# pcodec/pcodec

Measured on AMD Instinct MI355X. Metric: encode+decode GB/s (uncompressed) per chunk, u64/f64 2^18-elem, higher is better.
Workload: dtype u64

## Files before the change

### pcodec_amd/csrc/encode_fast.hip

```cpp
#pragma once

namespace pcogfx {

constexpr uint32_t kRunBatches = 64;

struct EncFast {
  uint8_t* sym;
  uint16_t* answ;
  uint32_t* bat;
  uint64_t* run_start;
  uint32_t* fstate;
  uint16_t* vlut;
  uint32_t bat_stride, run_stride;
  uint32_t runs_per_page, fused;
  uint64_t stride;
  uint64_t* body;
  uint32_t* wp_block;
};
__device__ __forceinline__ uint64_t fast_at(const EncPage PCO_GLOBAL* pg, uint32_t skip) { return uni((uint64_t)pg->start) + skip + 16ull * uni(pg->page_idx); }

__device__ __forceinline__ uint8_t PCO_GLOBAL* fsym_ptr(const EncWorkspace& ws, const EncFast& fx, uint32_t task, uint32_t var) {
  return (uint8_t PCO_GLOBAL*)fx.sym + ((uint64_t)task * ws.n_slots + ws.slot_of_var[var]) * fx.stride;
}
__device__ __forceinline__ uint16_t PCO_GLOBAL* fansw_ptr(const EncWorkspace& ws, const EncFast& fx, uint32_t task, uint32_t var) {
  return (uint16_t PCO_GLOBAL*)fx.answ + ((uint64_t)task * ws.n_slots + ws.slot_of_var[var]) * fx.stride;
}

struct PageVar { uint32_t present, n_bins, asl, max_ob, needs_ans, trivial, skip, n_lat, compact; uint64_t minv, rel, range; };
__device__ __forceinline__ PageVar page_var(const EncChunk PCO_GLOBAL* ch, uint32_t v, uint32_t page_n) {
  PageVar r;
  r.present = uni(ch->v[v].present); r.n_bins = uni(ch->v[v].n_bins); r.asl = uni(ch->v[v].ans_size_log); r.max_ob = uni(ch->v[v].max_ob);
  r.needs_ans = uni(ch->v[v].needs_ans); r.trivial = uni(ch->v[v].is_trivial);
// ... 628 lines not shown
  uint64_t bits = kBitsModeVariant;
  if (mode_kind == kIntMult || mode_kind == kFloatMult) bits += LB; else if (mode_kind == kFloatQuant) bits += kBitsQuantK;
  if (uni(ch->dict_dtype)) bits = 32 + 8ull * uni(ch->dict_k) * (uint32_t)(dtype_bits(uni(ch->dict_dtype)) / 8);
  bits += kBitsDeltaVariant;
  if (delta_kind == kDeltaConsecutive) bits += kBitsDeltaOrder + 1;
  else if (delta_kind == kDeltaLookback) bits += kBitsLookbackWindowLog + kBitsLookbackStateLog + 1;
  else if (delta_kind == kDeltaConv1) bits += 5 + 64 + 5 + 32ull * uni(ch->delta_order);
  for (int v = 0; v < 3; v++) {
    if (!uni(ch->v[v].present)) continue;
    const uint32_t lb = v == 0 ? 32u : LB;
    bits += kBitsAnsSizeLog + kBitsNBins + (uint64_t)uni(ch->v[v].n_bins) * (uni(ch->v[v].ans_size_log) + lb + offset_bits_bits(lb));
  }
  return (bits + 7) & ~(uint64_t)7;
}

__global__ __launch_bounds__(64) void enc_scan_kernel(EncWorkspace ws, EncFast fx, PcoGfxTaskResult* results, uint32_t n_pages) {
  const uint32_t p = blockIdx.x;
  if (p >= n_pages) return;
  const uint32_t lane = lane_id();
  EncPage PCO_GLOBAL* pg = (EncPage PCO_GLOBAL*)ws.pages + p;
  const uint32_t t = uni(pg->chunk);
  EncChunk PCO_GLOBAL* ch = (EncChunk PCO_GLOBAL*)ws.chunks + t;
  if (!page_is_fast(ch, pg)) return;
  const uint32_t LB = (uint32_t)dtype_bits(uni(ch->dtype));
  const uint32_t page_n = (uint32_t)uni((uint64_t)pg->n);
  const uint32_t pflags = uni(pg->flags);
  PageVar pv[3]; uint32_t ob0[3];
  uint64_t head = 0;
  if (pflags & kPageFlagPreamble) head += 8 + kBitsNEntries + chunk_meta_bits_of(ch, LB);
  uint64_t page_meta = 0;
  const uint32_t delta_kind = uni(ch->delta_kind);
#pragma unroll
  for (int v = 0; v < 3; v++) {
    pv[v] = page_var(ch, v, page_n);
    ob0[v] = 0;
    if (!pv[v].present) continue;
    if (pv[v].n_bins == 1) ob0[v] = uni((uint32_t)plan_ref(ws, t, v).bob()[0]);
    if (v == 1) page_meta += (uint64_t)LB * ((delta_kind == kDeltaConsecutive || delta_kind == kDeltaConv1) ? uni(ch->delta_order) : (delta_kind == kDeltaLookback ? (1u << uni(ch->state_n_log)) : 0u));
    page_meta += 4ull * pv[v].asl;
  }
  head += (page_meta + 7) & ~(uint64_t)7;
  uint32_t PCO_GLOBAL* dst32 = (uint32_t PCO_GLOBAL*)pg->dst;
  const uint64_t cap_bits = uni((uint64_t)pg->dst_cap) * 8;
  const uint32_t n_batches = (page_n + kBatchN - 1) / kBatchN;
  if (fx.body != nullptr) {
    const uint64_t rec = uni(fx.body[2ull * p]);
    if (rec >> 63) {
      const uint64_t end = head + (rec & ~(1ull << 63)), total = (end + 7) & ~(uint64_t)7;
      const bool overflow = total + 64 > cap_bits;
      if (lane == 0) {
        pg->pad = overflow ? 1u : (0x100u | (15u << 4));
        store_result((PcoGfxTaskResult PCO_GLOBAL*)results + p, overflow ? 0 : total >> 3, overflow ? PCO_GFX_INVALID_ARGUMENT : PCO_GFX_OK, 0);
        if (!overflow) { dst32[0] = 0; dst32[total >> 5] = 0; dst32[end >> 5] = 0; dst32[head >> 5] = 0; fx.run_start[(uint64_t)p * fx.run_stride] = head; }
      }
      return;
    }
  }
  uint64_t carry = head;
  for (int pass = 0; pass < 2; pass++) {
    carry = head;
    for (uint32_t c0 = 0; c0 < n_batches; c0 += 64) {
      const uint32_t b = c0 + lane;
      uint64_t bits = 0;
      if (b < n_batches) {
        const uint32_t base = b * kBatchN;
#pragma unroll
        for (int v = 0; v < 3; v++) {
          if (!pv[v].present || pv[v].trivial || base >= pv[v].n_lat) continue;
// ... 471 lines not shown
  if (kWide && (uint32_t)dtype_bits(uni(ch->dtype)) != LBits<L>::v) return;
  PageVar pv[3];
#pragma unroll
  for (int v = 0; v < 3; v++) pv[v] = page_var(ch, v, page_n);
  pack1_run<L, kMask, kWide>(ws, fx, p, run, pg, t, pv, page_n);
}

__global__ __launch_bounds__(64) void enc_pack_kernel(EncWorkspace ws, EncFast fx, uint32_t n_pages) {
  const uint32_t p = blockIdx.x / fx.runs_per_page, run = blockIdx.x % fx.runs_per_page;
  if (p >= n_pages) return;
  EncPage PCO_GLOBAL* pg = (EncPage PCO_GLOBAL*)ws.pages + p;
  EncChunk PCO_GLOBAL* ch = (EncChunk PCO_GLOBAL*)ws.chunks + uni(pg->chunk);
  const uint32_t pad = uni(pg->pad);
  if (!page_is_fast(ch, pg) || (pad & 1u) != 0) return;
  const bool lean = ((pad >> 4) & 0xfu) != 0;
  if (lean && run != 0) return;
  const int bits = dtype_bits(uni(ch->dtype));
  if (bits == 64) pack_run<uint64_t>(ws, fx, p, run, pg, ch, lean);
  else if (bits == 32) pack_run<uint32_t>(ws, fx, p, run, pg, ch, lean);
  else if (bits == 16) pack_run<uint16_t>(ws, fx, p, run, pg, ch, lean);
  else pack_run<uint8_t>(ws, fx, p, run, pg, ch, lean);
}

}
```

### pcodec_amd/csrc/encode_walkpack.hip

```cpp
#pragma once

namespace pcogfx {

constexpr uint32_t kWpWaves = 6;
constexpr uint32_t kWpQ = 16, kWpHelpers = 8, kWpH = kWpQ / kWpHelpers;
constexpr uint32_t kWpSlot = 5120;
constexpr uint32_t kWpStgDwords = 132;
constexpr uint32_t kWpSkew = 8, kWpSlotUse = kWpSlot - kWpSkew * (16 - 1);
__device__ __forceinline__ uint32_t wp_slot(uint32_t q) { return q * (kWpSlot + kWpSkew); }
constexpr uint32_t kWpStgOff = (kWpSlotUse - kWpStgDwords * 4) & ~15u;
constexpr uint32_t kWpAnsOff = kWpStgOff - 1024;
constexpr uint32_t kWpSymOff = kWpAnsOff - 512;
constexpr uint32_t kWpLdsBytes = kWpQ * kWpSlot;
static_assert(kWpStgOff % 16 == 0 && kWpAnsOff % 16 == 0 && kWpSymOff % 16 == 0 && kWpStgOff + kWpStgDwords * 4 <= kWpSlotUse, "aligned sections");
static_assert(2 * kWpLdsBytes <= 160 * 1024, "two blocks per CU");
constexpr uint64_t kWpBodyFlag = 1ull << 63;
__device__ __forceinline__ bool wp_fits(uint32_t asl, uint32_t n_bins) { return ew_info_off(asl) + 12u * n_bins <= kWpSymOff; }

__device__ __forceinline__ void wp_put(uint32_t stg_addr, uint32_t pos, uint64_t val) {
  const uint32_t dw = pos >> 5, sh = pos & 31;
  const uint64_t lo = val << sh;
  uint32_t PCO_LDS* s = (uint32_t PCO_LDS*)(uintptr_t)(stg_addr + 4u * dw);
  const uint32_t hi = (uint32_t)((val >> 1) >> (63 - sh));
  atomicOr((uint32_t*)&s[0], (uint32_t)lo);
// ... 5 lines not shown

__device__ __forceinline__ PageVar page_var_lane(const EncChunk PCO_GLOBAL* ch, uint32_t v, uint32_t page_n) {
  PageVar r;
  r.present = ch->v[v].present; r.n_bins = ch->v[v].n_bins; r.asl = ch->v[v].ans_size_log; r.max_ob = ch->v[v].max_ob;
  r.needs_ans = ch->v[v].needs_ans; r.trivial = ch->v[v].is_trivial;
  r.skip = v == 2 ? 0u : ch->v[v].lat_start;
  if (r.skip > page_n) r.skip = page_n;
  r.n_lat = page_n - r.skip;
  r.compact = ch->v[v].hist_path == 0 ? 1u : 0u;
  r.minv = (uint64_t)ch->v[v].minv;
  r.range = (uint64_t)ch->v[v].maxv - r.minv;
  r.rel = v != 0 && ch->c16_ok == 1 ? ch->c16_ref[v == 2 ? 1 : 0] : r.minv;
  return r;
}

__global__ __launch_bounds__(64 * (1 + kWpHelpers)) __attribute__((amdgpu_waves_per_eu(kWpWaves, kWpWaves))) void enc_walkp_kernel(EncWorkspace ws, EncFast fx, uint32_t n_pages) {
  const uint32_t lane = lane_id(), wave = threadIdx.x >> 6;
  uint8_t PCO_LDS* smem = enc_lds_base();
  const uint32_t lds0 = (uint32_t)(uintptr_t)smem;
  const uint32_t n_items = n_pages * ws.n_slots;
  typedef uint64_t __attribute__((aligned(2))) u64_align2;
  const uint32_t iq = lane & 15u, sub = lane >> 4;
  const uint32_t l_item = blockIdx.x * kWpQ + iq;
  const bool l_exists = l_item < n_items;
  const uint32_t l_p = l_exists ? l_item / ws.n_slots : 0u, l_sl = l_exists ? l_item % ws.n_slots : 0u;
  const uint32_t l_v = ws.slot_of_var[0] == l_sl ? 0u : (ws.slot_of_var[1] == l_sl ? 1u : 2u);
  const EncPage PCO_GLOBAL* l_pg = (const EncPage PCO_GLOBAL*)ws.pages + l_p;
  const uint32_t l_t = l_pg->chunk;
  const EncChunk PCO_GLOBAL* l_ch = (const EncChunk PCO_GLOBAL*)ws.chunks + l_t;
  const bool l_fast = l_exists && l_ch->status == PCO_GFX_OK && l_ch->fast_ok != 0 && !(l_pg->flags & kPageFlagMetaOnly);
  const uint32_t l_page_n = (uint32_t)l_pg->n;
  const PageVar l_pv = page_var_lane(l_ch, l_v, l_page_n);
  const bool l_writes = l_fast && l_pv.present && !l_pv.trivial;
  bool l_bad = false;
  if (l_writes) {
    if (l_v != 1 || !wd_walks(fx.fused, l_pv) || ws_walks(fx.fused, l_pv) || !wd_takes(fx.fused, l_pv) || !l_pv.needs_ans || l_pv.n_bins > 256 || !wp_fits(l_pv.asl, l_pv.n_bins)) l_bad = true;
    else if ((l_ch->v[0].present && !l_ch->v[0].is_trivial) || (l_ch->v[2].present && !l_ch->v[2].is_trivial)) l_bad = true;
  }
  {
    uint32_t worst = 0;
    if (l_writes && !l_bad) {
      const PlanRef plan = plan_ref(ws, l_t, l_v);
      for (uint32_t b = sub; b < l_pv.n_bins; b += 4) { const uint32_t w = ((plan.syminfo()[b] >> 14) & 15u) + 1u + plan.bob()[b]; worst = w > worst ? w : worst; }
    }
    { const uint32_t o = (uint32_t)__shfl_xor((int)worst, 16, 64); worst = worst > o ? worst : o; }
    { const uint32_t o = (uint32_t)__shfl_xor((int)worst, 32, 64); worst = worst > o ? worst : o; }
    if (worst > 16u) l_bad = true;
  }
  const bool ok = (fx.fused & kFusedLookups) != 0 && !__any(l_bad);
  if (threadIdx.x == 0) fx.wp_block[blockIdx.x] = ok ? 1u : 0u;
  if (!ok) {
    if (threadIdx.x < kWpQ) {
      const uint32_t item = blockIdx.x * kWpQ + threadIdx.x;
      if (item < n_items && ws.slot_of_var[1] == item % ws.n_slots) fx.body[2ull * (item / ws.n_slots)] = 0;
    }
    return;
  }
  const uint32_t l_nb = l_writes ? (l_pv.n_lat + kBatchN - 1) / kBatchN : 0u;
  const uint32_t max_nb = wave_max_u32(l_nb);
  if (l_fast && !l_writes && sub == 0 && wave == 0) {
    if (l_pv.present && (l_pv.n_bins <= 1 || l_pv.n_lat == 0)) for (uint32_t jj = 0; jj < 4; jj++) fx.fstate[((uint64_t)l_p * 3 + l_v) * 4 + jj] = 1u << l_pv.asl;
    if (l_v == 1) fx.body[2ull * l_p] = 0;
  }
  const uint32_t l_info_off = ew_info_off(l_pv.asl), l_cpk_off = l_info_off + 8u * l_pv.n_bins;
// ... 304 lines not shown
```

### pcodec_amd/csrc/pco_gfx.hip

```cpp
#include "pco_host.h"
#include "pco_half.h"

#include <algorithm>
#include <atomic>
#include <chrono>
#include <thread>
#include <mutex>
#include <condition_variable>
#include <functional>
#include <sched.h>
#include <pthread.h>
#include <sys/syscall.h>
#include <unistd.h>
#include <cstdlib>
#include <cstring>
#include <memory>
#include <unordered_map>

#include "pco_auto_host.inc"
#include "decode_kernel.hip"
#include "decode_trail.hip"
#include "encode_kernels.hip"
#include "encode_lookback.hip"
#include "encode_conv1.hip"
#include "encode_dict.hip"
#include "encode_hist_select.hip"
#include "encode_hist_literal.hip"
#include "auto_mode_kernels.hip"
#include "encode_fast.hip"
#include "encode_walkseg.hip"
#include "encode_walkpack.hip"
#include "stream_kernels.hip"
#include "stream_wrapped.hip"

namespace pcogfx {

static thread_local HostError g_err{PCO_GFX_OK, ""};
void set_error(int status, const std::string& msg) { g_err.status = status; g_err.msg = msg; }
void clear_error() { g_err.status = PCO_GFX_OK; g_err.msg.clear(); }

struct WorkspaceHolder {
  std::unordered_map<int, std::unique_ptr<Workspace>> by_device;
  ~WorkspaceHolder() {
    const bool worker = (long)syscall(SYS_gettid) != (long)getpid();
    for (auto& kv : by_device) {
      if (worker) { int cur = 0; const bool sw = hipGetDevice(&cur) == hipSuccess && cur != kv.first && hipSetDevice(kv.first) == hipSuccess; kv.second->release_all(); if (kv.second->last_event) (void)hipEventDestroy(kv.second->last_event); if (sw) (void)hipSetDevice(cur); }
// ... 521 lines not shown
```

### pcodec_amd/csrc/pco_gfx_encode_api.inc

```
namespace pcogfx {

struct ResolvedConfig {
  uint32_t level;
  uint32_t mode_kind; double mode_f64; uint64_t mode_u64;
  uint32_t delta_kind, delta_order;
  uint64_t max_page_n; bool enable_8_bit;
  bool strict_hist;
  bool conv1 = false;
  bool dict = false;
  DictTask* d_dict = nullptr;
  uint32_t unknown_flags = 0;
};

static bool g_strict_hist_env = env_is_one("PCO_GFX_STRICT_HISTOGRAM");
static ResolvedConfig resolve_config(const PcoChunkConfigEx* c) {
  ResolvedConfig r{8, PCO_MODE_AUTO, 0.0, 0, PCO_DELTA_AUTO, 0, 1u << 18, true, g_strict_hist_env};
  if (c) {
    r.level = c->compression_level; r.mode_kind = c->mode_kind; r.mode_f64 = c->mode_f64; r.mode_u64 = c->mode_u64;
    r.delta_kind = c->delta_kind; r.delta_order = c->delta_order; r.max_page_n = c->max_page_n ? c->max_page_n : (1u << 18);
    r.enable_8_bit = c->enable_8_bit != 0;
    r.strict_hist = g_strict_hist_env || (c->flags & PCO_GFX_CFG_STRICT_HISTOGRAM) != 0;
    r.conv1 = (c->flags & PCO_GFX_CFG_CONV1) != 0;
    r.dict = (c->flags & PCO_GFX_CFG_DICT) != 0;
    r.unknown_flags = c->flags & ~(uint32_t)(PCO_GFX_CFG_STRICT_HISTOGRAM | PCO_GFX_CFG_CONV1 | PCO_GFX_CFG_DICT);
// ... 140 lines not shown
  PCO_HIP_CHECK(hipMemcpyAsync(d_plans, plans.data(), n_tasks * sizeof(EncModePlan), hipMemcpyHostToDevice, stream));
  PCO_HIP_CHECK(hipMemcpyAsync(ws.pages, pages.data(), n_pages * sizeof(EncPage), hipMemcpyHostToDevice, stream));
  const uint32_t nt = (uint32_t)n_tasks, np = (uint32_t)n_pages;
  uint32_t skip_fast = 0;
  const uint32_t c16_enable = stop_after != 1 ? 1u : 0u;
  PCO_TIMED_LAUNCH("enc_init_kernel", stream, enc_init_kernel, dim3((nt + 63) / 64), dim3(64), 0, stream, ws, d_tasks, d_plans, nt, cfg.level, c16_enable);
  const uint32_t tiles_per_page = (uint32_t)std::max<uint64_t>((page_max + kSplitTile - 1) / kSplitTile, 1);
  if ((uint64_t)np * tiles_per_page >= (1ull << 31)) throw HostError{PCO_GFX_INVALID_ARGUMENT, "too many pages in one call"};
  bool any_full0 = !c16_enable, any_spec = c16_enable != 0;
  size_t n_lookback = 0;
  for (size_t i = 0; i < n_tasks; i++) n_lookback += plans[i].delta_kind == kDeltaLookback;
  any_full0 = any_full0 || n_lookback != 0 || any_big;
  if (c16_enable) PCO_TIMED_LAUNCH("enc_presample_kernel", stream, enc_presample_kernel, dim3(nt), dim3(64), 0, stream, ws, d_tasks, nt);
  PCO_TIMED_LAUNCH("enc_lat_slots_kernel", stream, enc_lat_slots_kernel, dim3((nt + 63) / 64), dim3(64), 0, stream, ws, nt, 0u);
  uint32_t n_full = 0;
  if (lat_exact) {
    uint32_t flags[3] = {0, 0, 0};
    PCO_HIP_CHECK(hipMemcpyAsync(flags, ws.need_sort, 12, hipMemcpyDeviceToHost, stream));
    PCO_HIP_CHECK(hipStreamSynchronize(stream));
    n_full = flags[2];
    any_full0 = n_full != 0; any_spec = c16_enable && n_full < n_tasks;
    ws.lat_cap1 = std::max<uint32_t>(n_full, 1u);
    ws.lat = (uint8_t*)wsp.enc_lat.ensure((size_t)ws.lat_cap1 * lat_slot_bytes);
    ws.lat2 = ws.lat;
  } else if (c16_enable) any_full0 = true;
  if (any_spec) PCO_TIMED_LAUNCH("enc_split_kernel<c16>", stream, (enc_split_kernel<true, false>), dim3(np * tiles_per_page), dim3(256), kSplitLdsBytes, stream, ws, d_tasks, tiles_per_page, 1u, 1u);
  if (any_full0) PCO_TIMED_LAUNCH("enc_split_kernel", stream, (enc_split_kernel<false, false>), dim3(np * tiles_per_page), dim3(256), kSplitLdsBytes, stream, ws, d_tasks, tiles_per_page, 1u, 0u);
  if (any_spec) {
    PCO_TIMED_LAUNCH("enc_lat_slots_kernel", stream, enc_lat_slots_kernel, dim3((nt + 63) / 64), dim3(64), 0, stream, ws, nt, 2u);
    bool any_redo = true;
    if (lat_exact) {
      uint32_t used = 0;
      PCO_HIP_CHECK(hipMemcpyAsync(&used, ws.lat_used, 4, hipMemcpyDeviceToHost, stream));
      PCO_HIP_CHECK(hipStreamSynchronize(stream));
      const uint32_t n_redo = used > ws.lat_cap1 ? used - ws.lat_cap1 : 0u;
      any_redo = used > n_full;
      if (n_redo) ws.lat2 = (uint8_t*)wsp.enc_lat2.ensure((size_t)n_redo * lat_slot_bytes);
    }
    if (any_redo) {
      const uint32_t tpb = 32, bpp = (tiles_per_page + tpb - 1) / tpb;
      PCO_TIMED_LAUNCH("enc_split_kernel(redo)", stream, (enc_split_kernel<false, true>), dim3(np * bpp), dim3(256), kSplitLdsBytes, stream, ws, d_tasks, tiles_per_page, tpb, 2u);
    }
  }
  if (stop_after == 1) { PCO_HIP_CHECK(hipGetLastError()); if (ws_out) *ws_out = ws; return; }
  if (any_conv1) {
    const size_t conv_bytes = (n_tasks * sizeof(EncConv) + 255) & ~(size_t)255;
    uint8_t* d_conv = (uint8_t*)wsp.enc_conv.ensure(conv_bytes + n_pages * kConv1MaxOrder * sizeof(uint32_t) + 256);
    ws.conv = (EncConv*)d_conv; ws.conv_state = (uint32_t*)(d_conv + conv_bytes);
    PCO_TIMED_LAUNCH("enc_conv1_stats_kernel", stream, enc_conv1_stats_kernel, dim3(nt), dim3(kConv1Threads), 0, stream, ws, nt);
// ... 37 lines not shown
  {
    static const bool wide_ok = hipFuncSetAttribute((const void*)enc_hist_wide_kernel<kWideHistRange>, hipFuncAttributeMaxDynamicSharedMemorySize, (int)hist_lds_bytes(kWideHistRange)) == hipSuccess &&
                                hipFuncSetAttribute((const void*)enc_hist_wide_kernel<kMidHistRange>, hipFuncAttributeMaxDynamicSharedMemorySize, (int)hist_lds_bytes(kMidHistRange)) == hipSuccess;
    if (!wide_ok) throw HostError{PCO_GFX_DEVICE_ERROR, "cannot reserve LDS for enc_hist_wide_kernel"};
    static const bool sort_ok = hipFuncSetAttribute((const void*)enc_hist_sort_kernel, hipFuncAttributeMaxDynamicSharedMemorySize, (int)kHistSortLdsBytes) == hipSuccess;
    if (!sort_ok) throw HostError{PCO_GFX_DEVICE_ERROR, "cannot reserve LDS for enc_hist_sort_kernel"};
    uint64_t max_n = 0; uint32_t small_lds = 0;
    for (size_t i = 0; i < n_tasks; i++) {
      max_n = std::max<uint64_t>(max_n, tasks[i].n);
      const uint32_t kb = dtype_bits(tasks[i].dtype) == 64 ? 8u : 4u;
      small_lds = std::max(small_lds, small_lds_bytes((uint32_t)std::min<uint64_t>(tasks[i].n, kSmallHistCap), kb));
    }
    const bool any_long = max_n > kSmallHistCap;
    bool run_mid = any_long, run_wide = any_long, run_sort = any_long || any_big, run_small = true;
    if (results != nullptr && stop_after == 0) {
      uint32_t flag = 0;
      PCO_HIP_CHECK(hipMemcpyAsync(&flag, ws.need_sort, 4, hipMemcpyDeviceToHost, stream));
      PCO_HIP_CHECK(hipStreamSynchronize(stream));
      run_sort = (flag & 1u) != 0; run_mid = (flag & 2u) != 0; run_wide = (flag & 4u) != 0; run_small = (flag & 8u) != 0;
    }
    if (run_sort && !sort_upfront) ws.sort = (uint8_t*)wsp.enc_sort.ensure(sort_bytes);
    if (run_mid || run_wide || run_small || run_sort) ws.walk = (uint8_t*)wsp.enc_walk.ensure((size_t)nt * 3 * kWalkRecBytes);
    if (run_mid) PCO_TIMED_LAUNCH("enc_hist_wide_kernel<16384>", stream, enc_hist_wide_kernel<kMidHistRange>, dim3(nt), dim3(1024), hist_lds_bytes(kMidHistRange), stream, ws, nt);
    if (run_wide) PCO_TIMED_LAUNCH("enc_hist_wide_kernel<32768>", stream, enc_hist_wide_kernel<kWideHistRange>, dim3(nt), dim3(1024), hist_lds_bytes(kWideHistRange), stream, ws, nt);
    if (run_small) {
      static const bool small_ok = hipFuncSetAttribute((const void*)enc_hist_small_kernel, hipFuncAttributeMaxDynamicSharedMemorySize, (int)small_lds_bytes(kSmallHistCap, 8)) == hipSuccess;
      if (!small_ok) throw HostError{PCO_GFX_DEVICE_ERROR, "cannot reserve LDS for enc_hist_small_kernel"};
      PCO_TIMED_LAUNCH("enc_hist_small_kernel", stream, enc_hist_small_kernel, dim3(nt), dim3(kSelT), small_lds, stream, ws, nt);
    }
    if (run_sort) {
      auto launch_sel = [&](auto kernel, const char* name) {
        if (hipFuncSetAttribute((const void*)kernel, hipFuncAttributeMaxDynamicSharedMemorySize, (int)kSelLdsBytes) != hipSuccess) throw HostError{PCO_GFX_DEVICE_ERROR, "cannot reserve LDS for enc_hist_select_kernel"};
        PCO_TIMED_LAUNCH(name, stream, kernel, dim3(nt), dim3(kSelThr), kSelLdsBytes, stream, ws, nt);
// ... 36 lines not shown
    fx.run_start = (uint64_t*)wsp.enc_run.ensure(n_pages * (size_t)fx.run_stride * 8);
    const size_t fstate_bytes = (n_pages * 12 * 4 + 63) & ~(size_t)63, body_bytes = (n_pages * 16 + 63) & ~(size_t)63, wpb_bytes = ((n_pages * (size_t)ws.n_slots + 15) / 16) * 4 + 64;
    fx.fstate = (uint32_t*)wsp.enc_fstate.ensure(fstate_bytes + body_bytes + wpb_bytes);
    const uint64_t n_blocks = (uint64_t)np * fx.runs_per_page;
    if (n_blocks < (1ull << 31)) {
      const uint32_t n_items = np * ws.n_slots;
      const size_t vlut_bytes = n_tasks * (size_t)ws.n_slots * kDirectHistRange * 2;
      uint64_t input_bytes = 0; for (size_t i = 0; i < n_tasks; i++) input_bytes += tasks[i].n * (uint64_t)(dtype_bits(tasks[i].dtype) / 8);
      const bool lookups = vlut_bytes <= std::max<uint64_t>(64ull << 20, input_bytes / 2);
      static const bool walkp_on = env_not_zero("PCO_GFX_WALKP");
      const bool keep_fused = walkp_on && lookups && ws.n_slots == 1;
      fx.fused = n_items > 8192 && !keep_fused ? 2u : 1u;
      if (lookups) fx.fused |= kFusedLookups;
      const bool any_seg = page_max >= (uint64_t)kWsMinBatches * kBatchN && n_items <= kWsMaxItems;
      if (any_seg) fx.fused |= kFusedSegments;
      PCO_TIMED_LAUNCH("enc_dissect_kernel", stream, enc_dissect_kernel, dim3(np * ((fx.runs_per_page + kDisRuns - 1) / kDisRuns)), dim3(256), kDisLdsBytes, stream, ws, fx, np);
      if (fx.fused & kFusedLookups) {
        fx.vlut = (uint16_t*)wsp.enc_vlut.ensure(vlut_bytes + 64);
        PCO_TIMED_LAUNCH("enc_vlut_kernel", stream, enc_vlut_kernel, dim3(nt * 3), dim3(256), 0, stream, ws, fx, nt);
      }
      static const bool walkd_ok = hipFuncSetAttribute((const void*)enc_walkd_kernel, hipFuncAttributeMaxDynamicSharedMemorySize, (int)kWdLdsBytes) == hipSuccess;
      if (!walkd_ok) throw HostError{PCO_GFX_DEVICE_ERROR, "cannot reserve LDS for enc_walkd_kernel"};
      if (any_seg) PCO_TIMED_LAUNCH("enc_walkseg_kernel", stream, enc_walkseg_kernel, dim3(n_items), dim3(128), kWsLdsBytes, stream, ws, fx, np);
      if (walkp_on && !any_seg && (fx.fused & kFusedLookups) != 0) {
        static const bool walkp_ok = hipFuncSetAttribute((const void*)enc_walkp_kernel, hipFuncAttributeMaxDynamicSharedMemorySize, (int)kWpLdsBytes) == hipSuccess;
        if (!walkp_ok) throw HostError{PCO_GFX_DEVICE_ERROR, "cannot reserve LDS for enc_walkp_kernel"};
        fx.body = (uint64_t*)((uint8_t*)fx.fstate + fstate_bytes); fx.wp_block = (uint32_t*)((uint8_t*)fx.fstate + fstate_bytes + body_bytes);
        PCO_TIMED_LAUNCH("enc_walkp_kernel", stream, enc_walkp_kernel, dim3((n_items + kWpQ - 1) / kWpQ), dim3(64 * (1 + kWpHelpers)), kWpLdsBytes, stream, ws, fx, np);
      }
      PCO_TIMED_LAUNCH("enc_walkd_kernel", stream, enc_walkd_kernel, dim3((n_items + kWdQ - 1) / kWdQ), dim3(64 * (1 + kWdHelpers)), kWdLdsBytes, stream, ws, fx, np);
      if ((fx.fused & 0xffu) == 2u) PCO_TIMED_LAUNCH("enc_walk16_kernel", stream, enc_walk_kernel<16>, dim3((n_items + 15) / 16), dim3(64), EwCfg<16>::kLdsBytes, stream, ws, fx, np, 1u);
      PCO_TIMED_LAUNCH("enc_scan_kernel", stream, enc_scan_kernel, dim3(np), dim3(64), 0, stream, ws, fx, d_results, np);
      const bool forked = fx.body != nullptr;
      std::unique_ptr<ScopedKernelTimer> span;
      if (forked) {
        ensure_side_stream(wsp);
        span.reset(new ScopedKernelTimer("enc_place+pack", stream));
        PCO_HIP_CHECK(hipEventRecord(wsp.fork_event, stream));
        PCO_HIP_CHECK(hipStreamWaitEvent(wsp.side_stream, wsp.fork_event, 0));
        PCO_TIMED_LAUNCH("~enc_place_kernel", wsp.side_stream, enc_place_kernel, dim3(np * place_pieces(page_max)), dim3(256), 0, wsp.side_stream, ws, fx, np, place_pieces(page_max));
        PCO_HIP_CHECK(hipEventRecord(wsp.join_event, wsp.side_stream));
      }
      bool any1 = false, any_sec = false, any_lb = false, any32 = false, any64 = false;
      for (size_t i = 0; i < n_tasks; i++) {
        const bool sec = plans[i].mode_kind != kClassic, lb = plans[i].delta_kind == kDeltaLookback;
        any_sec |= sec; any_lb |= lb; any1 |= !sec && !lb;
// ... 1251 lines not shown
```

### pcodec_amd/csrc/pco_host.h

```cpp
#pragma once
#include <hip/hip_runtime.h>
#include <stdint.h>

#include <algorithm>
#include <cstdlib>
#include <string>
#include <vector>

#include "../../include/pco_gfx.h"

namespace pcogfx {

struct HostError {
  int status;
  std::string msg;
  bool oom = false;
};

void set_error(int status, const std::string& msg);
void clear_error();

inline bool env_is_one(const char* name) { const char* e = std::getenv(name); return e != nullptr && e[0] == '1'; }
inline bool env_not_zero(const char* name) { const char* e = std::getenv(name); return !(e != nullptr && e[0] == '0'); }
inline char env_char(const char* name) { const char* e = std::getenv(name); return e != nullptr ? e[0] : '\0'; }
// ... 46 lines not shown
  DevBuf dec_stats;
  hipStream_t side_stream = nullptr, side_stream2 = nullptr; hipEvent_t fork_event = nullptr, join_event = nullptr, join_event2 = nullptr;
  int n_cus = 0;
  DevBuf dec_hist;
  DevBuf io_in, io_out;
  DevBuf compact_tasks;
  DevBuf enc_state;
  DevBuf enc_lat, enc_lat2, enc_sort, enc_ans, enc_small, enc_lb, enc_walk;
  DevBuf enc_lbprops;
  DevBuf enc_sym, enc_answ, enc_bat, enc_run, enc_fstate, enc_vlut;
  DevBuf enc_strict;
  DevBuf enc_conv;
  DevBuf enc_dict, enc_dict_hbm;
  DevBuf auto_idx, auto_samp, auto_tasks, auto_sum, auto_log2;
  HostBuf h_samp, h_sum;
#define PCO_WS_BUFS(X) X(tasks) X(results) X(tbl_ws) X(dec_plans) X(dec_bins) X(dec_sym) X(dec_offpos) X(dec_progress) X(dec_stats) X(dec_hist) X(io_in) X(io_out) X(compact_tasks) X(enc_state) \
  X(enc_lat) X(enc_lat2) X(enc_sort) X(enc_ans) X(enc_small) X(enc_lb) X(enc_lbprops) X(enc_walk) X(enc_sym) X(enc_answ) X(enc_bat) X(enc_run) X(enc_fstate) X(enc_vlut) X(enc_strict) X(enc_conv) X(enc_dict) X(enc_dict_hbm) X(auto_idx) X(auto_samp) X(auto_tasks) X(auto_sum) X(auto_log2)
  size_t device_bytes() const {
    size_t b = 0;
#define PCO_WS_ADD(name) b += name.cap;
    PCO_WS_BUFS(PCO_WS_ADD)
#undef PCO_WS_ADD
    return b;
  }
  std::string device_report() const {
    std::string r;
#define PCO_WS_REP(name) if (name.cap) r += std::string(#name) + "=" + std::to_string(name.cap) + " ";
    PCO_WS_BUFS(PCO_WS_REP)
#undef PCO_WS_REP
    return r;
  }
  unsigned long long acc_givebacks = 0, acc_marked = 0, acc_strict = 0;
  void fold_counters() {
    uint32_t v[2] = {0, 0};
    if (dec_stats.p && hipMemcpy(v, dec_stats.p, 8, hipMemcpyDeviceToHost) == hipSuccess) { acc_givebacks += v[0]; acc_marked += v[1]; }
    uint32_t f = 0;
    if (enc_strict.p && hipMemcpy(&f, enc_strict.p, 4, hipMemcpyDeviceToHost) == hipSuccess) acc_strict += f;
  }
  void release_all() {
    fold_counters();
    if (side_stream) { (void)hipStreamSynchronize(side_stream); (void)hipStreamDestroy(side_stream); side_stream = nullptr; }
    if (side_stream2) { (void)hipStreamSynchronize(side_stream2); (void)hipStreamDestroy(side_stream2); side_stream2 = nullptr; }
    if (fork_event) { (void)hipEventDestroy(fork_event); fork_event = nullptr; }
    if (join_event) { (void)hipEventDestroy(join_event); join_event = nullptr; }
    if (join_event2) { (void)hipEventDestroy(join_event2); join_event2 = nullptr; }
    tasks.release(); results.release(); tbl_ws.release(); dec_plans.release(); dec_bins.release(); dec_sym.release(); dec_offpos.release(); dec_progress.release(); dec_stats.release(); dec_hist.release(); io_in.release(); io_out.release(); compact_tasks.release();
    enc_state.release(); enc_lat.release(); enc_lat2.release(); enc_sort.release(); enc_ans.release(); enc_small.release(); enc_lb.release(); enc_lbprops.release(); enc_walk.release(); enc_sym.release(); enc_answ.release(); enc_bat.release(); enc_run.release(); enc_fstate.release(); enc_vlut.release(); enc_strict.release(); enc_conv.release(); enc_dict.release(); enc_dict_hbm.release(); auto_idx.release(); auto_samp.release(); auto_tasks.release(); auto_sum.release(); auto_log2.release(); h_samp.release(); h_sum.release();
  }
};
Workspace& workspace();
struct WorkspaceUse {
  Workspace& ws; hipStream_t stream;
  WorkspaceUse(Workspace& w, hipStream_t s) : ws(w), stream(s) {
    if (ws.has_last && ws.last_stream != stream && ws.last_event) (void)hipStreamWaitEvent(stream, ws.last_event, 0);
  }
  ~WorkspaceUse() {
    if (!ws.last_event && hipEventCreateWithFlags(&ws.last_event, hipEventDisableTiming) != hipSuccess) { ws.last_event = nullptr; return; }
    if (hipEventRecord(ws.last_event, stream) == hipSuccess) { ws.last_stream = stream; ws.has_last = true; }
  }
};

struct HostBitWriter {
// ... 25 lines not shown
```

Measured before the change: 1731.

## Write page headers early on side stream and overlap host readbacks with split launch

Adds an enc_head_kernel that writes each page's header (preamble, chunk metadata, delta moments) on a side stream while the walk kernels run. enc_scan then ORs the final ANS states into the header with atomics, and enc_pack skips lean pages when head_early is set. The host readback of sort flags now goes into pinned memory tracked by an event, so the c16 split kernel can be queued before the host waits. This removes a serial pack launch and some host stall, at the cost of an extra kernel, cross-stream events, and atomics that only work if the header dwords are pre-zeroed correctly.

```diff
diff --git a/pcodec_amd/csrc/encode_fast.hip b/pcodec_amd/csrc/encode_fast.hip
--- a/pcodec_amd/csrc/encode_fast.hip
+++ b/pcodec_amd/csrc/encode_fast.hip
@@ -16,6 +16,8 @@
   uint64_t stride;
   uint64_t* body;
   uint32_t* wp_block;
+  uint32_t head_early;
+  uint32_t pad_head;
 };
 __device__ __forceinline__ uint64_t fast_at(const EncPage PCO_GLOBAL* pg, uint32_t skip) { return uni((uint64_t)pg->start) + skip + 16ull * uni(pg->page_idx); }
 
@@ -674,6 +676,22 @@
   return (bits + 7) & ~(uint64_t)7;
 }
 
+struct HeadBits { uint64_t pre, head; uint32_t nlps; };
+__device__ __forceinline__ HeadBits page_head_bits(const EncChunk PCO_GLOBAL* ch, uint32_t pflags, uint32_t LB) {
+  HeadBits h;
+  h.pre = (pflags & kPageFlagPreamble) ? 8 + kBitsNEntries + chunk_meta_bits_of(ch, LB) : 0ull;
+  const uint32_t delta_kind = uni(ch->delta_kind);
+  h.nlps = (delta_kind == kDeltaConsecutive || delta_kind == kDeltaConv1) ? uni(ch->delta_order) : (delta_kind == kDeltaLookback ? (1u << uni(ch->state_n_log)) : 0u);
+  uint64_t page_meta = 0;
+  for (int v = 0; v < 3; v++) {
+    if (!uni(ch->v[v].present)) continue;
+    if (v == 1) page_meta += (uint64_t)LB * h.nlps;
+    page_meta += 4ull * uni(ch->v[v].ans_size_log);
+  }
+  h.head = h.pre + ((page_meta + 7) & ~(uint64_t)7);
+  return h;
+}
+
 __global__ __launch_bounds__(64) void enc_scan_kernel(EncWorkspace ws, EncFast fx, PcoGfxTaskResult* results, uint32_t n_pages) {
   const uint32_t p = blockIdx.x;
   if (p >= n_pages) return;
@@ -686,20 +704,14 @@
   const uint32_t page_n = (uint32_t)uni((uint64_t)pg->n);
   const uint32_t pflags = uni(pg->flags);
   PageVar pv[3]; uint32_t ob0[3];
-  uint64_t head = 0;
-  if (pflags & kPageFlagPreamble) head += 8 + kBitsNEntries + chunk_meta_bits_of(ch, LB);
-  uint64_t page_meta = 0;
-  const uint32_t delta_kind = uni(ch->delta_kind);
+  const HeadBits hb = page_head_bits(ch, pflags, LB);
+  const uint64_t head = hb.head;
 #pragma unroll
   for (int v = 0; v < 3; v++) {
     pv[v] = page_var(ch, v, page_n);
     ob0[v] = 0;
-    if (!pv[v].present) continue;
-    if (pv[v].n_bins == 1) ob0[v] = uni((uint32_t)plan_ref(ws, t, v).bob()[0]);
-    if (v == 1) page_meta += (uint64_t)LB * ((delta_kind == kDeltaConsecutive || delta_kind == kDeltaConv1) ? uni(ch->delta_order) : (delta_kind == kDeltaLookback ? (1u << uni(ch->state_n_log)) : 0u));
-    page_meta += 4ull * pv[v].asl;
-  }
-  head += (page_meta + 7) & ~(uint64_t)7;
+    if (pv[v].present && pv[v].n_bins == 1) ob0[v] = uni((uint32_t)plan_ref(ws, t, v).bob()[0]);
+  }
   uint32_t PCO_GLOBAL* dst32 = (uint32_t PCO_GLOBAL*)pg->dst;
   const uint64_t cap_bits = uni((uint64_t)pg->dst_cap) * 8;
   const uint32_t n_batches = (page_n + kBatchN - 1) / kBatchN;
@@ -708,10 +720,31 @@
     if (rec >> 63) {
       const uint64_t end = head + (rec & ~(1ull << 63)), total = (end + 7) & ~(uint64_t)7;
       const bool overflow = total + 64 > cap_bits;
+      const bool early = fx.head_early != 0;
       if (lane == 0) {
         pg->pad = overflow ? 1u : (0x100u | (15u << 4));
         store_result((PcoGfxTaskResult PCO_GLOBAL*)results + p, overflow ? 0 : total >> 3, overflow ? PCO_GFX_INVALID_ARGUMENT : PCO_GFX_OK, 0);
-        if (!overflow) { dst32[0] = 0; dst32[total >> 5] = 0; dst32[end >> 5] = 0; dst32[head >> 5] = 0; fx.run_start[(uint64_t)p * fx.run_stride] = head; }
+        if (!overflow) {
+          if (!early) { dst32[0] = 0; dst32[total >> 5] = 0; dst32[end >> 5] = 0; dst32[head >> 5] = 0; }
+          else { if ((total >> 5) > (head >> 5)) dst32[total >> 5] = 0; if ((end >> 5) > (head >> 5)) dst32[end >> 5] = 0; }
+          fx.run_start[(uint64_t)p * fx.run_stride] = head;
+        }
+      }
+      if (early && !overflow) {
+        uint64_t spos = hb.pre;
+#pragma unroll
+        for (int v = 0; v < 3; v++) {
+          if (!pv[v].present) continue;
+          if (v == 1) spos += (uint64_t)LB * hb.nlps;
+          const uint32_t asl = pv[v].asl;
+          if ((lane >> 2) == (uint32_t)v && asl != 0) {
+            const uint64_t at = spos + (uint64_t)(lane & 3u) * asl;
+            const uint64_t val = (uint64_t)((fx.fstate[((uint64_t)p * 3 + v) * 4 + (lane & 3u)] - (1u << asl)) & ((1u << asl) - 1u)) << (at & 31);
+            atomicOr((uint32_t*)(dst32 + (at >> 5)), (uint32_t)val);
+            if (val >> 32) atomicOr((uint32_t*)(dst32 + (at >> 5) + 1), (uint32_t)(val >> 32));
+          }
+          spos += 4ull * asl;
+        }
       }
       return;
     }
@@ -1213,6 +1246,7 @@
   const uint32_t pad = uni(pg->pad);
   if (!page_is_fast(ch, pg) || (pad & 1u) != 0) return;
   const bool lean = ((pad >> 4) & 0xfu) != 0;
+  if (((pad >> 4) & 0xfu) == 15u && fx.head_early != 0) return;
   if (lean && run != 0) return;
   const int bits = dtype_bits(uni(ch->dtype));
   if (bits == 64) pack_run<uint64_t>(ws, fx, p, run, pg, ch, lean);
diff --git a/pcodec_amd/csrc/encode_head.hip b/pcodec_amd/csrc/encode_head.hip
--- /dev/null
+++ b/pcodec_amd/csrc/encode_head.hip
@@ -0,0 +1,80 @@
+#pragma once
+
+namespace pcogfx {
+
+__device__ __forceinline__ uint32_t head_part(uint64_t val, uint64_t pos, uint32_t nbits, uint64_t lo) {
+  const int64_t rel = (int64_t)(pos - lo);
+  if (rel >= 32 || rel + (int64_t)nbits <= 0) return 0u;
+  if (nbits < 64) val &= ((uint64_t)1 << nbits) - 1;
+  return rel >= 0 ? (uint32_t)(val << rel) : (uint32_t)(val >> (uint32_t)(-rel));
+}
+
+__global__ __launch_bounds__(64) __attribute__((amdgpu_waves_per_eu(8, 8))) void enc_head_kernel(EncWorkspace ws, EncFast fx, uint32_t n_pages) {
+  const uint32_t p = blockIdx.x, lane = lane_id();
+  if (p >= n_pages) return;
+  {
+    const uint32_t item = p * ws.n_slots + ws.slot_of_var[1];
+    const WpLane wl = wp_inspect(ws, fx, item / kWpQ, n_pages * ws.n_slots, lane);
+    const uint32_t mine = wl.writes && wl.pv.n_lat != 0 ? 1u : 0u;
+    if (!wl.ok || __builtin_amdgcn_readlane((int)mine, (int)uni(item % kWpQ)) == 0) return;
+  }
+  const EncPage PCO_GLOBAL* pg = (const EncPage PCO_GLOBAL*)ws.pages + p;
+  const uint32_t t = uni(pg->chunk);
+  const EncChunk PCO_GLOBAL* ch = (const EncChunk PCO_GLOBAL*)ws.chunks + t;
+  const uint32_t LB = (uint32_t)dtype_bits(uni(ch->dtype));
+  const uint32_t page_n = (uint32_t)uni((uint64_t)pg->n), pflags = uni(pg->flags);
+  const HeadBits hb = page_head_bits(ch, pflags, LB);
+  if (hb.head + 64 > uni((uint64_t)pg->dst_cap) * 8) return;
+  const uint32_t mode_kind = uni(ch->mode_kind), delta_kind = uni(ch->delta_kind), dict_dtype = uni(ch->dict_dtype);
+  auto dword_at = [&](uint64_t lo) {
+    uint32_t w = 0; uint64_t pos = 0;
+    auto put = [&](uint64_t val, uint32_t nbits) { w |= head_part(val, pos, nbits, lo); pos += nbits; };
+    if (pflags & kPageFlagPreamble) {
+      put(dict_dtype ? dict_dtype : uni(ch->dtype), 8);
+      put(page_n - 1, kBitsNEntries);
+      if (dict_dtype) {
+        put(kDict, kBitsModeVariant); put(uni(ch->dict_k), kBitsDictLen);
+        pos = ((pos + 7) & ~(uint64_t)7) + 8ull * uni(ch->dict_k) * ((uint32_t)dtype_bits(dict_dtype) / 8);
+      } else put(mode_kind, kBitsModeVariant);
+      if (mode_kind == kIntMult || mode_kind == kFloatMult) put(uni((uint64_t)ch->mode_base), LB);
+      else if (mode_kind == kFloatQuant) put(uni(ch->mode_k), kBitsQuantK);
+      put(delta_kind, kBitsDeltaVariant);
+      if (delta_kind == kDeltaConsecutive) { put(uni(ch->delta_order), kBitsDeltaOrder); put(0, 1); }
+      else if (delta_kind == kDeltaLookback) { put(uni(ch->window_n_log) - 1, kBitsLookbackWindowLog); put(uni(ch->state_n_log), kBitsLookbackStateLog); put(0, 1); }
+      else if (delta_kind == kDeltaConv1) {
+        const EncConv PCO_GLOBAL* cv = (const EncConv PCO_GLOBAL*)ws.conv + t;
+        const uint32_t order = uni(cv->order);
+        put(uni(cv->quant), 5); put(uni((uint64_t)cv->bias) ^ (1ull << 63), 64); put(order - 1, 5);
+        for (uint32_t k = 0; k < order; k++) put((uint32_t)uni((uint64_t)cv->w[k]) ^ 0x80000000u, 32);
+      }
+      for (uint32_t v = 0; v < 3; v++) {
+        if (!uni(ch->v[v].present)) continue;
+        const uint32_t asl = uni(ch->v[v].ans_size_log), n_bins = uni(ch->v[v].n_bins);
+        const uint32_t lb = v == 0 ? 32u : LB, obb = offset_bits_bits(lb), bin_bits = asl + lb + obb;
+        put(asl, kBitsAnsSizeLog); put(n_bins, kBitsNBins);
+        const uint64_t sect = (uint64_t)n_bins * bin_bits;
+        if (lo + 32 > pos && lo < pos + sect) {
+          const PlanRef plan = plan_ref(ws, t, v);
+          for (uint32_t b = lo > pos ? (uint32_t)(lo - pos) / bin_bits : 0u; b < n_bins; b++) {
+            const uint64_t at = pos + (uint64_t)b * bin_bits;
+            if (at >= lo + 32) break;
+            w |= head_part(plan.bweight()[b] - 1, at, asl, lo) | head_part(plan.blower()[b], at + asl, lb, lo) | head_part(plan.bob()[b], at + asl + lb, obb, lo);
+          }
+        }
+        pos += sect;
+      }
+      pos = (pos + 7) & ~(uint64_t)7;
+    }
+    if (uni(ch->v[1].present)) {
+      pos += uni(ch->v[0].present) ? 4ull * uni(ch->v[0].ans_size_log) : 0ull;
+      if (delta_kind == kDeltaConv1) { const uint32_t PCO_GLOBAL* st = (const uint32_t PCO_GLOBAL*)ws.conv_state + (uint64_t)p * kConv1MaxOrder; for (uint32_t i = 0; i < hb.nlps; i++) put(uni(st[i]), LB); }
+      else for (uint32_t i = 0; i < hb.nlps; i++) put(uni((uint64_t)pg->moments[i]), LB);
+    }
+    return w;
+  };
+  uint32_t PCO_GLOBAL* dst32 = (uint32_t PCO_GLOBAL*)pg->dst;
+  const uint32_t last = (uint32_t)(hb.head >> 5);
+  for (uint32_t d = lane; d <= last; d += 64) dst32[d] = dword_at(32ull * d);
+}
+
+}
diff --git a/pcodec_amd/csrc/encode_walkpack.hip b/pcodec_amd/csrc/encode_walkpack.hip
--- a/pcodec_amd/csrc/encode_walkpack.hip
+++ b/pcodec_amd/csrc/encode_walkpack.hip
@@ -43,14 +43,15 @@
   return r;
 }
 
-__global__ __launch_bounds__(64 * (1 + kWpHelpers)) __attribute__((amdgpu_waves_per_eu(kWpWaves, kWpWaves))) void enc_walkp_kernel(EncWorkspace ws, EncFast fx, uint32_t n_pages) {
-  const uint32_t lane = lane_id(), wave = threadIdx.x >> 6;
-  uint8_t PCO_LDS* smem = enc_lds_base();
-  const uint32_t lds0 = (uint32_t)(uintptr_t)smem;
-  const uint32_t n_items = n_pages * ws.n_slots;
-  typedef uint64_t __attribute__((aligned(2))) u64_align2;
+struct WpLane {
+  bool ok;
+  bool fast, writes;
+  uint32_t p, v, t;
+  const EncPage PCO_GLOBAL* pg; PageVar pv;
+};
+__device__ __forceinline__ WpLane wp_inspect(const EncWorkspace& ws, const EncFast& fx, uint32_t block, uint32_t n_items, uint32_t lane) {
   const uint32_t iq = lane & 15u, sub = lane >> 4;
-  const uint32_t l_item = blockIdx.x * kWpQ + iq;
+  const uint32_t l_item = block * kWpQ + iq;
   const bool l_exists = l_item < n_items;
   const uint32_t l_p = l_exists ? l_item / ws.n_slots : 0u, l_sl = l_exists ? l_item % ws.n_slots : 0u;
   const uint32_t l_v = ws.slot_of_var[0] == l_sl ? 0u : (ws.slot_of_var[1] == l_sl ? 1u : 2u);
@@ -76,7 +77,25 @@
     { const uint32_t o = (uint32_t)__shfl_xor((int)worst, 32, 64); worst = worst > o ? worst : o; }
     if (worst > 16u) l_bad = true;
   }
-  const bool ok = (fx.fused & kFusedLookups) != 0 && !__any(l_bad);
+  WpLane r;
+  r.ok = (fx.fused & kFusedLookups) != 0 && !__any(l_bad);
+  r.fast = l_fast; r.writes = l_writes; r.p = l_p; r.v = l_v; r.t = l_t; r.pg = l_pg; r.pv = l_pv;
+  return r;
+}
+
+__global__ __launch_bounds__(64 * (1 + kWpHelpers)) __attribute__((amdgpu_waves_per_eu(kWpWaves, kWpWaves))) void enc_walkp_kernel(EncWorkspace ws, EncFast fx, uint32_t n_pages) {
+  const uint32_t lane = lane_id(), wave = threadIdx.x >> 6;
+  uint8_t PCO_LDS* smem = enc_lds_base();
+  const uint32_t lds0 = (uint32_t)(uintptr_t)smem;
+  const uint32_t n_items = n_pages * ws.n_slots;
+  typedef uint64_t __attribute__((aligned(2))) u64_align2;
+  const uint32_t sub = lane >> 4;
+  const WpLane wl = wp_inspect(ws, fx, blockIdx.x, n_items, lane);
+  const bool ok = wl.ok;
+  const bool l_fast = wl.fast, l_writes = wl.writes;
+  const uint32_t l_p = wl.p, l_v = wl.v, l_t = wl.t;
+  const EncPage PCO_GLOBAL* l_pg = wl.pg;
+  const PageVar l_pv = wl.pv;
   if (threadIdx.x == 0) fx.wp_block[blockIdx.x] = ok ? 1u : 0u;
   if (!ok) {
     if (threadIdx.x < kWpQ) {
diff --git a/pcodec_amd/csrc/pco_gfx.hip b/pcodec_amd/csrc/pco_gfx.hip
--- a/pcodec_amd/csrc/pco_gfx.hip
+++ b/pcodec_amd/csrc/pco_gfx.hip
@@ -30,6 +30,7 @@
 #include "encode_fast.hip"
 #include "encode_walkseg.hip"
 #include "encode_walkpack.hip"
+#include "encode_head.hip"
 #include "stream_kernels.hip"
 #include "stream_wrapped.hip"
 
diff --git a/pcodec_amd/csrc/pco_gfx_encode_api.inc b/pcodec_amd/csrc/pco_gfx_encode_api.inc
--- a/pcodec_amd/csrc/pco_gfx_encode_api.inc
+++ b/pcodec_amd/csrc/pco_gfx_encode_api.inc
@@ -178,25 +178,32 @@
   if (c16_enable) PCO_TIMED_LAUNCH("enc_presample_kernel", stream, enc_presample_kernel, dim3(nt), dim3(64), 0, stream, ws, d_tasks, nt);
   PCO_TIMED_LAUNCH("enc_lat_slots_kernel", stream, enc_lat_slots_kernel, dim3((nt + 63) / 64), dim3(64), 0, stream, ws, nt, 0u);
   uint32_t n_full = 0;
+  volatile uint32_t* h_flags = lat_exact ? (volatile uint32_t*)wsp.h_flags.ensure(64) : nullptr;
+  bool split16_queued = false;
   if (lat_exact) {
-    uint32_t flags[3] = {0, 0, 0};
-    PCO_HIP_CHECK(hipMemcpyAsync(flags, ws.need_sort, 12, hipMemcpyDeviceToHost, stream));
-    PCO_HIP_CHECK(hipStreamSynchronize(stream));
-    n_full = flags[2];
+    if (!wsp.readback_event) PCO_HIP_CHECK(hipEventCreateWithFlags(&wsp.readback_event, hipEventDisableTiming));
+    PCO_HIP_CHECK(hipMemcpyAsync((void*)h_flags, ws.need_sort, 12, hipMemcpyDeviceToHost, stream));
+    PCO_HIP_CHECK(hipEventRecord(wsp.readback_event, stream));
+    if (c16_enable) {
+      PCO_TIMED_LAUNCH("enc_split_kernel<c16>", stream, (enc_split_kernel<true, false>), dim3(np * tiles_per_page), dim3(256), kSplitLdsBytes, stream, ws, d_tasks, tiles_per_page, 1u, 1u);
+      split16_queued = true;
+    }
+    PCO_HIP_CHECK(hipEventSynchronize(wsp.readback_event));
+    n_full = h_flags[2];
     any_full0 = n_full != 0; any_spec = c16_enable && n_full < n_tasks;
     ws.lat_cap1 = std::max<uint32_t>(n_full, 1u);
     ws.lat = (uint8_t*)wsp.enc_lat.ensure((size_t)ws.lat_cap1 * lat_slot_bytes);
     ws.lat2 = ws.lat;
   } else if (c16_enable) any_full0 = true;
-  if (any_spec) PCO_TIMED_LAUNCH("enc_split_kernel<c16>", stream, (enc_split_kernel<true, false>), dim3(np * tiles_per_page), dim3(256), kSplitLdsBytes, stream, ws, d_tasks, tiles_per_page, 1u, 1u);
+  if (any_spec && !split16_queued) PCO_TIMED_LAUNCH("enc_split_kernel<c16>", stream, (enc_split_kernel<true, false>), dim3(np * tiles_per_page), dim3(256), kSplitLdsBytes, stream, ws, d_tasks, tiles_per_page, 1u, 1u);
   if (any_full0) PCO_TIMED_LAUNCH("enc_split_kernel", stream, (enc_split_kernel<false, false>), dim3(np * tiles_per_page), dim3(256), kSplitLdsBytes, stream, ws, d_tasks, tiles_per_page, 1u, 0u);
   if (any_spec) {
     PCO_TIMED_LAUNCH("enc_lat_slots_kernel", stream, enc_lat_slots_kernel, dim3((nt + 63) / 64), dim3(64), 0, stream, ws, nt, 2u);
     bool any_redo = true;
     if (lat_exact) {
-      uint32_t used = 0;
-      PCO_HIP_CHECK(hipMemcpyAsync(&used, ws.lat_used, 4, hipMemcpyDeviceToHost, stream));
+      PCO_HIP_CHECK(hipMemcpyAsync((void*)(h_flags + 4), ws.lat_used, 4, hipMemcpyDeviceToHost, stream));
       PCO_HIP_CHECK(hipStreamSynchronize(stream));
+      const uint32_t used = h_flags[4];
       const uint32_t n_redo = used > ws.lat_cap1 ? used - ws.lat_cap1 : 0u;
       any_redo = used > n_full;
       if (n_redo) ws.lat2 = (uint8_t*)wsp.enc_lat2.ensure((size_t)n_redo * lat_slot_bytes);
@@ -264,9 +271,9 @@
     const bool any_long = max_n > kSmallHistCap;
     bool run_mid = any_long, run_wide = any_long, run_sort = any_long || any_big, run_small = true;
     if (results != nullptr && stop_after == 0) {
-      uint32_t flag = 0;
-      PCO_HIP_CHECK(hipMemcpyAsync(&flag, ws.need_sort, 4, hipMemcpyDeviceToHost, stream));
+      PCO_HIP_CHECK(hipMemcpyAsync((void*)(h_flags + 5), ws.need_sort, 4, hipMemcpyDeviceToHost, stream));
       PCO_HIP_CHECK(hipStreamSynchronize(stream));
+      const uint32_t flag = h_flags[5];
       run_sort = (flag & 1u) != 0; run_mid = (flag & 2u) != 0; run_wide = (flag & 4u) != 0; run_small = (flag & 8u) != 0;
     }
     if (run_sort && !sort_upfront) ws.sort = (uint8_t*)wsp.enc_sort.ensure(sort_bytes);
@@ -333,6 +340,16 @@
       if (lookups) fx.fused |= kFusedLookups;
       const bool any_seg = page_max >= (uint64_t)kWsMinBatches * kBatchN && n_items <= kWsMaxItems;
       if (any_seg) fx.fused |= kFusedSegments;
+      const bool walkp = walkp_on && !any_seg && (fx.fused & kFusedLookups) != 0;
+      if (walkp) {
+        fx.body = (uint64_t*)((uint8_t*)fx.fstate + fstate_bytes); fx.wp_block = (uint32_t*)((uint8_t*)fx.fstate + fstate_bytes + body_bytes);
+        fx.head_early = 1;
+        ensure_side_stream(wsp);
+        PCO_HIP_CHECK(hipEventRecord(wsp.fork_event, stream));
+        PCO_HIP_CHECK(hipStreamWaitEvent(wsp.side_stream, wsp.fork_event, 0));
+        PCO_TIMED_LAUNCH("~enc_head_kernel", wsp.side_stream, enc_head_kernel, dim3(np), dim3(64), 0, wsp.side_stream, ws, fx, np);
+        PCO_HIP_CHECK(hipEventRecord(wsp.join_event, wsp.side_stream));
+      }
       PCO_TIMED_LAUNCH("enc_dissect_kernel", stream, enc_dissect_kernel, dim3(np * ((fx.runs_per_page + kDisRuns - 1) / kDisRuns)), dim3(256), kDisLdsBytes, stream, ws, fx, np);
       if (fx.fused & kFusedLookups) {
         fx.vlut = (uint16_t*)wsp.enc_vlut.ensure(vlut_bytes + 64);
@@ -341,14 +358,14 @@
       static const bool walkd_ok = hipFuncSetAttribute((const void*)enc_walkd_kernel, hipFuncAttributeMaxDynamicSharedMemorySize, (int)kWdLdsBytes) == hipSuccess;
       if (!walkd_ok) throw HostError{PCO_GFX_DEVICE_ERROR, "cannot reserve LDS for enc_walkd_kernel"};
       if (any_seg) PCO_TIMED_LAUNCH("enc_walkseg_kernel", stream, enc_walkseg_kernel, dim3(n_items), dim3(128), kWsLdsBytes, stream, ws, fx, np);
-      if (walkp_on && !any_seg && (fx.fused & kFusedLookups) != 0) {
+      if (walkp) {
         static const bool walkp_ok = hipFuncSetAttribute((const void*)enc_walkp_kernel, hipFuncAttributeMaxDynamicSharedMemorySize, (int)kWpLdsBytes) == hipSuccess;
         if (!walkp_ok) throw HostError{PCO_GFX_DEVICE_ERROR, "cannot reserve LDS for enc_walkp_kernel"};
-        fx.body = (uint64_t*)((uint8_t*)fx.fstate + fstate_bytes); fx.wp_block = (uint32_t*)((uint8_t*)fx.fstate + fstate_bytes + body_bytes);
         PCO_TIMED_LAUNCH("enc_walkp_kernel", stream, enc_walkp_kernel, dim3((n_items + kWpQ - 1) / kWpQ), dim3(64 * (1 + kWpHelpers)), kWpLdsBytes, stream, ws, fx, np);
       }
       PCO_TIMED_LAUNCH("enc_walkd_kernel", stream, enc_walkd_kernel, dim3((n_items + kWdQ - 1) / kWdQ), dim3(64 * (1 + kWdHelpers)), kWdLdsBytes, stream, ws, fx, np);
       if ((fx.fused & 0xffu) == 2u) PCO_TIMED_LAUNCH("enc_walk16_kernel", stream, enc_walk_kernel<16>, dim3((n_items + 15) / 16), dim3(64), EwCfg<16>::kLdsBytes, stream, ws, fx, np, 1u);
+      if (walkp) PCO_HIP_CHECK(hipStreamWaitEvent(stream, wsp.join_event, 0));
       PCO_TIMED_LAUNCH("enc_scan_kernel", stream, enc_scan_kernel, dim3(np), dim3(64), 0, stream, ws, fx, d_results, np);
       const bool forked = fx.body != nullptr;
       std::unique_ptr<ScopedKernelTimer> span;
diff --git a/pcodec_amd/csrc/pco_host.h b/pcodec_amd/csrc/pco_host.h
--- a/pcodec_amd/csrc/pco_host.h
+++ b/pcodec_amd/csrc/pco_host.h
@@ -84,6 +84,8 @@
   DevBuf enc_dict, enc_dict_hbm;
   DevBuf auto_idx, auto_samp, auto_tasks, auto_sum, auto_log2;
   HostBuf h_samp, h_sum;
+  HostBuf h_flags;
+  hipEvent_t readback_event = nullptr;
 #define PCO_WS_BUFS(X) X(tasks) X(results) X(tbl_ws) X(dec_plans) X(dec_bins) X(dec_sym) X(dec_offpos) X(dec_progress) X(dec_stats) X(dec_hist) X(io_in) X(io_out) X(compact_tasks) X(enc_state) \
   X(enc_lat) X(enc_lat2) X(enc_sort) X(enc_ans) X(enc_small) X(enc_lb) X(enc_lbprops) X(enc_walk) X(enc_sym) X(enc_answ) X(enc_bat) X(enc_run) X(enc_fstate) X(enc_vlut) X(enc_strict) X(enc_conv) X(enc_dict) X(enc_dict_hbm) X(auto_idx) X(auto_samp) X(auto_tasks) X(auto_sum) X(auto_log2)
   size_t device_bytes() const {
@@ -114,8 +116,9 @@
     if (fork_event) { (void)hipEventDestroy(fork_event); fork_event = nullptr; }
     if (join_event) { (void)hipEventDestroy(join_event); join_event = nullptr; }
     if (join_event2) { (void)hipEventDestroy(join_event2); join_event2 = nullptr; }
+    if (readback_event) { (void)hipEventDestroy(readback_event); readback_event = nullptr; }
     tasks.release(); results.release(); tbl_ws.release(); dec_plans.release(); dec_bins.release(); dec_sym.release(); dec_offpos.release(); dec_progress.release(); dec_stats.release(); dec_hist.release(); io_in.release(); io_out.release(); compact_tasks.release();
-    enc_state.release(); enc_lat.release(); enc_lat2.release(); enc_sort.release(); enc_ans.release(); enc_small.release(); enc_lb.release(); enc_lbprops.release(); enc_walk.release(); enc_sym.release(); enc_answ.release(); enc_bat.release(); enc_run.release(); enc_fstate.release(); enc_vlut.release(); enc_strict.release(); enc_conv.release(); enc_dict.release(); enc_dict_hbm.release(); auto_idx.release(); auto_samp.release(); auto_tasks.release(); auto_sum.release(); auto_log2.release(); h_samp.release(); h_sum.release();
+    enc_state.release(); enc_lat.release(); enc_lat2.release(); enc_sort.release(); enc_ans.release(); enc_small.release(); enc_lb.release(); enc_lbprops.release(); enc_walk.release(); enc_sym.release(); enc_answ.release(); enc_bat.release(); enc_run.release(); enc_fstate.release(); enc_vlut.release(); enc_strict.release(); enc_conv.release(); enc_dict.release(); enc_dict_hbm.release(); auto_idx.release(); auto_samp.release(); auto_tasks.release(); auto_sum.release(); auto_log2.release(); h_samp.release(); h_sum.release(); h_flags.release();
   }
 };
 Workspace& workspace();
```

After: 1752, median of 6. +1.2%, better.
